# Magicyw/Quadruped-PyMPC-TAMOLS

Hardware: AMD Instinct MI355X
Metric: SRBD rollouts/sec + p50 MPC-step ms at N=10k H=12; 1/2/4/8 GPU (higher is better)
Workload: dtype f32; 1 GPU; go2_trot_flat_mppi_n10000_h12_zo; num_samples=10000, rows_per_gpu=10000, horizon=12, method=mppi, parametrization=zero_order, robot=go2, gait=trot, parallelism=single GPU

## Files before the change

### quadruped-pympc-tamols_amd/csrc/srbd_device.h

```cpp
#pragma once

#include <utility>

#include "srbd_jaxrng.h"
#include "srbd_launch.h"

namespace srbd {

#ifdef SRBD_ROLLOUT_STAMPS
constexpr int RSTAMP_N = 6, RSTAMP_BLOCKS = 8192;
__device__ uint64_t g_rstamp[RSTAMP_BLOCKS * RSTAMP_N];
#define SRBD_RSTAMP(i)                                                                  \
    do {                                                                                \
        if (threadIdx.x == 0 && blockIdx.x < RSTAMP_BLOCKS) {                           \
            asm volatile("s_waitcnt vmcnt(0) lgkmcnt(0)" ::: "memory");                 \
            g_rstamp[blockIdx.x * RSTAMP_N + (i)] = __builtin_amdgcn_s_memrealtime(); \
        }                                                                               \
    } while (0)
__device__ uint64_t g_lstamp[RSTAMP_BLOCKS * 8];
__device__ uint64_t g_fstamp[64];
#define SRBD_LSTAMP(i)                                                                            \
    do {                                                                                          \
        if (threadIdx.x == 0 && blockIdx.x < RSTAMP_BLOCKS)                                       \
            g_lstamp[blockIdx.x * 8 + (i)] = __builtin_amdgcn_s_memrealtime();                    \
// ... 219 lines not shown
    int q = first / n, k = first - q * n;
    const int sq = stride / n, sk = stride - sq * n;
    while (q < nq) {
        rng_item(mc, in->sigma, (uint32_t)seed, (uint32_t)(seed >> 32), (uint32_t)ctr, (uint32_t)(ctr >> 32), k, q,
                 job.noise);
        k += sk;
        q += sq;
        if (k >= n) {
            k -= n;
            ++q;
        }
    }
}

__host__ __device__ constexpr int chunk_index(int n, int H, int S) { return (n * S) / H; }

template <int N>
struct IntC {
    static constexpr int value = N;
};
template <class F, int... Ns>
__device__ __forceinline__ void unroll_seq(F&& f, std::integer_sequence<int, Ns...>) {
    (f(IntC<Ns>{}), ...);
}

__device__ __forceinline__ void st_rec(float* p, float v) {
    __hip_atomic_store(reinterpret_cast<uint32_t*>(p), __float_as_uint(v), __ATOMIC_RELAXED, __HIP_MEMORY_SCOPE_AGENT);
}
__device__ __forceinline__ float ld_rec(const float* p) {
    return __uint_as_float(
        __hip_atomic_load(reinterpret_cast<const uint32_t*>(p), __ATOMIC_RELAXED, __HIP_MEMORY_SCOPE_AGENT));
}
template <int U>
__device__ __forceinline__ void stage_recs16(const float* __restrict__ src, float* dst, int n) {
    const int tid = threadIdx.x, T = blockDim.x, n4 = n >> 2;
    const auto rs = __builtin_amdgcn_make_buffer_rsrc((void*)src, (short)0, n * 4, 0x00020000);
    float4* d4 = reinterpret_cast<float4*>(dst);
    for (int i0 = 0; i0 < n4; i0 += U * T) {
        float4 v[U];
#pragma unroll
        for (int u = 0; u < U; ++u) {
            const auto x = __builtin_amdgcn_raw_buffer_load_b128(rs, 16 * (i0 + u * T + tid), 0, 16);
            v[u] = make_float4(__uint_as_float(x[0]), __uint_as_float(x[1]), __uint_as_float(x[2]),
                               __uint_as_float(x[3]));
        }
#pragma unroll
        for (int u = 0; u < U; ++u) {
            const int i = i0 + u * T + tid;
            if (i < n4) d4[i] = v[u];
        }
    }
}
template <int U>
__device__ __forceinline__ void stage_recs(const float* __restrict__ src, float* dst, int n) {
    const int tid = threadIdx.x, T = blockDim.x, n2 = n >> 1;
    const uint64_t* s2 = reinterpret_cast<const uint64_t*>(src);
    uint64_t* d2 = reinterpret_cast<uint64_t*>(dst);
    for (int i0 = 0; i0 < n2; i0 += U * T) {
        uint64_t v[U];
#pragma unroll
        for (int u = 0; u < U; ++u) {
            const int i = i0 + u * T + tid;
            v[u] = i < n2 ? __hip_atomic_load(s2 + i, __ATOMIC_RELAXED, __HIP_MEMORY_SCOPE_AGENT) : 0ull;
        }
#pragma unroll
        for (int u = 0; u < U; ++u) {
            const int i = i0 + u * T + tid;
            if (i < n2) d2[i] = v[u];
        }
    }
}


__device__ __forceinline__ void fold_node_lds(const ModelConst& mc, const float* st, int rec_stride, int nb, float* G) {
    __shared__ float sc_sh[TREE_FAN];
    __shared__ float gh_sh[2];
    __shared__ uint64_t gk_sh[MAXK + 1];
    const int tid = threadIdx.x, T = blockDim.x;
    const int P = mc.P, K = mc.K;
    const bool rs = mc.method == SRBD_RANDOM_SAMPLING;
    if (tid < 64) {
        const float* R = st + (size_t)tid * rec_stride;
        const bool have = tid < nb;
        const float m = have ? R[0] : 0.0f;
        const uint32_t row = have ? __float_as_uint(R[2]) : 0u;
        const uint64_t key = have ? ((uint64_t)__float_as_uint(m) << 32) | row : KEY_NONE;
        const uint64_t gk = wave_min_u64(key);
        const float beta = __uint_as_float((uint32_t)(gk >> 32));
        if (key == gk) gh_sh[1] = R[3];
        if (tid == 0) {
            gh_sh[0] = beta;
            gk_sh[MAXK] = gk;
        }
        if (have) sc_sh[tid] = rs ? 1.0f : expf(-1.0f * (m - beta));
        if (tid == 0) gk_sh[0] = gk;
    }
    __syncthreads();
    SRBD_LSTAMP(4);
    if (!rs) {
        for (int j = tid; j <= P; j += T) {
            const int off = j < P ? REC_HDR + j : 1;
            float a = 0.0f;
            int cb = 0;
            for (; cb + 8 <= nb; cb += 8) {
                float x[8];
#pragma unroll
                for (int u = 0; u < 8; ++u) x[u] = st[(size_t)(cb + u) * rec_stride + off];
#pragma unroll
                for (int u = 0; u < 8; ++u) a = a + sc_sh[cb + u] * x[u];
            }
            for (; cb < nb; ++cb) a = a + sc_sh[cb] * st[(size_t)cb * rec_stride + off];
            st_rec(&G[off], a);
        }
    }
    SRBD_LSTAMP(5);
    if (tid == 0) {
        st_rec(&G[0], gh_sh[0]);
        if (rs) st_rec(&G[1], 1.0f);
        st_rec(&G[2], __uint_as_float((uint32_t)gk_sh[MAXK]));
        st_rec(&G[3], gh_sh[1]);
    }
    if (tid < K) {
        const uint64_t kk = gk_sh[tid];
        st_rec(&G[REC_HDR + P + 2 * tid], __uint_as_float((uint32_t)kk));
        st_rec(&G[REC_HDR + P + 2 * tid + 1], __uint_as_float((uint32_t)(kk >> 32)));
    }
}

__device__ __forceinline__ bool level1_fold(const ModelConst& mc, const float* __restrict__ recs, int rec_stride,
                                            const GroupArgs& grp, int nroll, int lpb, float* st) {
    __shared__ int last_sh;
    const int tid = threadIdx.x;
    const int bpg = TREE_FAN / lpb;
    const int g = (int)blockIdx.x / bpg;
    const int nblk = min(bpg, nroll - g * bpg);
    const int nb = min(TREE_FAN, mc.nleaf - g * TREE_FAN);
    SRBD_LSTAMP(0);
    asm volatile("s_waitcnt vmcnt(0)" ::: "memory");
    __syncthreads();
    SRBD_LSTAMP(1);
    if (tid == 0) {
        const uint32_t old = __hip_atomic_fetch_add(grp.cnt + g, 1u, __ATOMIC_RELAXED, __HIP_MEMORY_SCOPE_AGENT);
        last_sh = old == (uint32_t)(nblk - 1);
    }
    __syncthreads();
    if (!last_sh) return false;
    SRBD_LSTAMP(2);
    if (tid == 0) __hip_atomic_store(grp.cnt + g, 0u, __ATOMIC_RELAXED, __HIP_MEMORY_SCOPE_AGENT);
    stage_recs16<5>(recs + (size_t)g * TREE_FAN * rec_stride, st, nb * rec_stride);
    __syncthreads();
    SRBD_LSTAMP(3);
    fold_node_lds(mc, st, rec_stride, nb, grp.grecs + (size_t)g * rec_stride);
    return true;
}

template <int CTRL, int ROWMASK>
__device__ __forceinline__ float dpp_f32(float v) {
    return __int_as_float(__builtin_amdgcn_update_dpp(0, __float_as_int(v), CTRL, ROWMASK, 0xF, false));
}
template <int LEVELS>
__device__ __forceinline__ float lane_tree_f32(float v) {
    v = v + dpp_f32<0x111, 0xF>(v);
    v = v + dpp_f32<0x112, 0xF>(v);
    v = v + dpp_f32<0x114, 0xF>(v);
    v = v + dpp_f32<0x118, 0xF>(v);
    if constexpr (LEVELS >= 5) v = v + dpp_f32<0x142, 0xA>(v);
    if constexpr (LEVELS >= 6) v = v + dpp_f32<0x143, 0xC>(v);
    return v;
}
__device__ __forceinline__ float wave_sum_f32(float v) { return lane_tree_f32<6>(v); }

constexpr int REGEN_QUADS = 16;
template <int SPL, int RG>
__device__ __forceinline__ void leaf_wsum_lanes(const ModelConst& mc, const StepInput* __restrict__ in,
                                                const float* __restrict__ base, bool zs, const float* e_sh,
                                                float* rbuf, int rec_stride, int k0, int gen = 0) {
    constexpr int CB = SPL == 4 ? 8 : 12;
    constexpr int LPL = 64 / SPL;
    const int lane = threadIdx.x & 63, w = threadIdx.x >> 6, NW = blockDim.x >> 6;
    const int P = mc.P;
    const size_t ldn = (size_t)mc.ldn;
    float e[SPL];
#pragma unroll
    for (int u = 0; u < SPL; ++u) e[u] = e_sh[SPL * lane + u];
    float* rec = rbuf + (lane / LPL) * rec_stride;
    const bool writer = (lane % LPL) == LPL - 1;
    int jreg = 0;
    if constexpr (RG && SPL == 4) {
        if (RG == 2 || (mc.method == SRBD_MPPI && mc.rng == RNG_PHILOX && in->noise_scaled == 0 && 4 * REGEN_QUADS <= P)) {
            const uint32_t key0 = in->seed_lo, key1 = in->seed_hi, c2 = in->ctr_lo, c3 = in->ctr_hi;
            const int nq = RG == 2 ? gen - 1 : REGEN_QUADS;
            for (int q = w; q < nq; q += NW) {
                float zq[4][SPL];
#pragma unroll
                for (int u = 0; u < SPL; ++u) {
                    const int k = k0 + SPL * lane + u, r = mc.row0 + k;
                    uint32_t c[4] = {(uint32_t)(r - 1), (uint32_t)q, c2, c3};
                    philox4x32_10(c, key0, key1);
                    float v[4];
                    box_muller(c[0], c[1], v[0], v[1]);
                    box_muller(c[2], c[3], v[2], v[3]);
                    const bool live = r > 0 && k < mc.n_local;
#pragma unroll
                    for (int i = 0; i < 4; ++i) zq[i][u] = live ? mc.sigma_mppi * v[i] : 0.0f;
                }
#pragma unroll
                for (int i = 0; i < 4; ++i) {
                    float p[SPL];
#pragma unroll
                    for (int u = 0; u < SPL; ++u) p[u] = e[u] * (zq[i][u] * 1.0f);
                    float a = (p[0] + p[1]) + (p[2] + p[3]);
                    a = lane_tree_f32<4>(a);
                    if (writer) rec[REC_HDR + 4 * q + i] = a;
                }
            }
            jreg = 4 * nq;
        }
    }
    for (int j0 = jreg + w; j0 <= P; j0 += CB * NW) {
        float z[CB][SPL];
#pragma unroll
        for (int b = 0; b < CB; ++b) {
            const int j = j0 + b * NW;
            const float* col = base + (size_t)(j < P ? j : 0) * ldn + SPL * lane;
            if constexpr (SPL == 4) {
                const float4 v = *reinterpret_cast<const float4*>(col);
                z[b][0] = v.x, z[b][1] = v.y, z[b][2] = v.z, z[b][3] = v.w;
            } else {
                const float2 v = *reinterpret_cast<const float2*>(col);
                z[b][0] = v.x, z[b][1] = v.y;
            }
        }
#pragma unroll
        for (int b = 0; b < CB; ++b) {
            const int j = j0 + b * NW;
            if (j > P) break;
            float p[SPL];
            if (j < P) {
                const float sj = zs ? in->sigma[j] : 1.0f;
#pragma unroll
                for (int u = 0; u < SPL; ++u) p[u] = e[u] * (z[b][u] * sj);
            } else {
#pragma unroll
                for (int u = 0; u < SPL; ++u) p[u] = e[u];
            }
            float a;
            if constexpr (SPL == 4)
                a = (p[0] + p[1]) + (p[2] + p[3]);
            else
                a = p[0] + p[1];
            a = lane_tree_f32<SPL == 4 ? 4 : 5>(a);
            if (writer) rec[j < P ? REC_HDR + j : 1] = a;
        }
    }
}

template <bool ZS>
__device__ __forceinline__ void leaf_wsum_cols(const ModelConst& mc, const StepInput* __restrict__ in,
                                               const float* __restrict__ base, const float* zst, int zstride, bool zs,
                                               const float* e_sh, float* __restrict__ rec) {
    const int tid = threadIdx.x, T = blockDim.x, P = mc.P;
    const size_t ldn = (size_t)mc.ldn;
    if ((tid >> 6) == (T >> 6) - 1) {
        const float t = wave_sum_f32(e_sh[tid & 63]);
        if ((tid & 63) == 63) st_rec(&rec[1], t);
    }
    for (int j = tid; j < P; j += T) {
        const float sj = zs ? in->sigma[j] : 1.0f;
        float first = 0.0f, tot = 0.0f;
#pragma nounroll
        for (int h = 0; h < 2; ++h) {
            float lv[16];
            if constexpr (ZS) {
#pragma unroll
                for (int i = 0; i < 16; ++i) {
                    const int r = 32 * h + 2 * i;
                    lv[i] = e_sh[r] * (zst[r * zstride + j] * sj) + e_sh[r + 1] * (zst[(r + 1) * zstride + j] * sj);
                }
            } else {
                const float4* row = reinterpret_cast<const float4*>(base + (size_t)j * ldn) + 8 * h;
                float4 v[8];
#pragma unroll
                for (int i = 0; i < 8; ++i) v[i] = row[i];
#pragma unroll
                for (int i = 0; i < 8; ++i) {
                    const int r = 32 * h + 4 * i;
                    lv[2 * i] = e_sh[r] * (v[i].x * sj) + e_sh[r + 1] * (v[i].y * sj);
                    lv[2 * i + 1] = e_sh[r + 2] * (v[i].z * sj) + e_sh[r + 3] * (v[i].w * sj);
                }
            }
#pragma unroll
            for (int n = 8; n >= 1; n >>= 1)
#pragma unroll
                for (int i = 0; i < n; ++i) lv[i] = lv[2 * i] + lv[2 * i + 1];
            if (h == 0)
                first = lv[0];
            else
                tot = first + lv[0];
        }
        st_rec(&rec[REC_HDR + j], tot);
    }
}

template <bool CEMT, bool ZS = false, bool TF = false, int RG = 0>
__device__ __forceinline__ bool block_epilogue(const ModelConst& mc, const StepInput* __restrict__ in, const int SPB,
                                               int sib, bool valid, float cost, const float* __restrict__ noise,
                                               float* __restrict__ recs, int rec_stride, float tag,
                                               const GroupArgs& grp, int nroll, float* zst = nullptr,
                                               int zstride = 0) {
    __shared__ uint64_t ks[ZS ? 64 : 256];
    __shared__ float e_sh[ZS ? 64 : 256];
    __shared__ uint64_t lmin[4];
    __shared__ uint64_t lel[CEMT ? 4 : 1][CEMT ? MAXK : 1];
    __shared__ float rbuf[TF ? 4 * ((REC_HDR + MAXP + 2 * MAXK + 3) & ~3) : 1];
    const int tid = threadIdx.x, lane = tid & 63, w = tid >> 6;
    const int lpb = SPB >> 6;
    const int P = mc.P, K = mc.K;
    const int k0 = blockIdx.x * SPB;
    const bool rs = mc.method == SRBD_RANDOM_SAMPLING;
    const uint64_t key = (sib >= 0 && valid) ? cost_key(cost, (uint32_t)(mc.row0 + k0 + sib)) : KEY_NONE;
    if (sib >= 0) ks[sib] = key;
    __syncthreads();
    constexpr bool ONE = ZS && !CEMT;
    uint64_t m1 = KEY_NONE;
    if constexpr (ONE) {
        m1 = wave_min_u64(ks[lane]);
    } else if (w < lpb) {
        const uint64_t m = wave_min_u64(ks[64 * w + lane]);
        if (lane == 0) lmin[w] = m;
    }
    if constexpr (CEMT) {
        if (K > 1) {
            for (int i = tid; i < lpb * MAXK; i += (int)blockDim.x) lel[i / MAXK][i % MAXK] = KEY_NONE;
            __syncthreads();
            const int lps = (int)blockDim.x / SPB, part = tid & (lps - 1), s = tid / lps, b = s >> 6;
            const uint64_t mine = ks[s];
            const int span = 64 / lps, i0 = 64 * b + part * span;
            int cnt = 0;
            for (int i = 0; i < span; ++i) cnt += ks[i0 + i] < mine ? 1 : 0;
            if (lps >= 2) cnt += __builtin_amdgcn_mov_dpp(cnt, 0xB1, 0xF, 0xF, true);
            if (lps == 4) cnt += __builtin_amdgcn_mov_dpp(cnt, 0x4E, 0xF, 0xF, true);
            if (part == 0 && cnt < K) lel[b][cnt] = mine;
        }
    }
    if constexpr (!ONE) __syncthreads();
    SRBD_RSTAMP(3);
    if (!rs) {
        const uint64_t lm = ONE ? m1 : (sib >= 0 ? lmin[sib >> 6] : KEY_NONE);
        if (sib >= 0) e_sh[sib] = valid ? expf(-1.0f * (cost - u2f((uint32_t)(lm >> 32)))) : 0.0f;
        __syncthreads();
        const bool zs = CEMT && zs_scaled(mc, in);
        if (SPB == 64)
            leaf_wsum_cols<ZS>(mc, in, noise + k0, zst, zstride, zs, e_sh, recs + (size_t)blockIdx.x * rec_stride);
        else if constexpr (TF) {
            if (SPB == 128)
                leaf_wsum_lanes<2, RG>(mc, in, noise + k0, zs, e_sh, rbuf, rec_stride, k0);
            else
                leaf_wsum_lanes<4, RG>(mc, in, noise + k0, zs, e_sh, rbuf, rec_stride, k0, grp.gen);
        }
    }
    SRBD_RSTAMP(4);
    const bool via_lds = TF && SPB > 64;
    float* const grec = recs + (size_t)blockIdx.x * lpb * rec_stride;
    auto put = [&](int b, int off, float v) {
        if (via_lds)
            rbuf[b * rec_stride + off] = v;
        else
            st_rec(&grec[(size_t)b * rec_stride + off], v);
    };
    auto leafmin = [&](int b) { return ONE ? m1 : lmin[b]; };
    if (tid < lpb) {
        const uint64_t m = leafmin(tid);
        put(tid, 0, u2f((uint32_t)(m >> 32)));
        put(tid, 2, u2f((uint32_t)m));
        if (rs) put(tid, 1, 1.0f);
    }
    if (sib >= 0 && key == leafmin(sib >> 6)) put(sib >> 6, 3, tag);
    for (int i = tid; i < lpb * K; i += (int)blockDim.x) {
        const int b = i / K, q = i % K;
        uint64_t kk = leafmin(b);
        if constexpr (CEMT) kk = K > 1 ? lel[b][q] : kk;
        put(b, REC_HDR + P + 2 * q, u2f((uint32_t)kk));
        put(b, REC_HDR + P + 2 * q + 1, u2f((uint32_t)(kk >> 32)));
    }
    if (via_lds) {
        __syncthreads();
        for (int i = tid; i < lpb * rec_stride; i += (int)blockDim.x) st_rec(&grec[i], rbuf[i]);
    }
    if constexpr (!CEMT) {
        if (grp.gsize > 1) {
            if (grp.fast) return true;
            if constexpr (ZS) {
                return level1_fold(mc, recs, rec_stride, grp, nroll, lpb, zst);
            } else {
                __shared__ __attribute__((aligned(16))) float st[GROUP_LDS_FLOATS];
                return level1_fold(mc, recs, rec_stride, grp, nroll, lpb, st);
            }
        }
    }
    return false;
}

constexpr uint32_t GA_FREQ_LANE = 0x10000u;

__device__ __forceinline__ float ga_sample_freq(const ModelConst& mc, const StepInput* __restrict__ in, int k) {
    if (in->ga_explicit) return mc.ga_freq[k];
    const uint64_t seed = ((uint64_t)in->seed_hi << 32) | in->seed_lo;
    if (mc.rng != RNG_PHILOX)
        return in->ga_freqs[jax_choice_index((uint32_t)(seed >> 32), (uint32_t)seed, (uint64_t)(mc.row0 + k),
                                             (uint64_t)mc.N, (uint32_t)in->ga_nfreq, mc.rng == RNG_JAX)];
    uint32_t c[4] = {(uint32_t)(mc.row0 + k), GA_FREQ_LANE, in->ctr_lo, in->ctr_hi};
    philox4x32_10(c, (uint32_t)seed, (uint32_t)(seed >> 32));
    const uint32_t i = (uint32_t)(((uint64_t)c[0] * (uint32_t)in->ga_nfreq) >> 32);
    return in->ga_freqs[i];
}

__device__ __forceinline__ void ga_contact_masks(const StepInput* __restrict__ in, int H, float f, uint32_t mask[4]) {
    const float inc = in->ga_dt * f;
    float t[4];
#pragma unroll
    for (int l = 0; l < 4; ++l) {
        t[l] = in->ga_timing[l];
        mask[l] = 0u;
    }
    for (int n = 0; n < H; ++n)
#pragma unroll
        for (int l = 0; l < 4; ++l) {
            t[l] = t[l] >= 1.0f ? 0.0f : t[l];
            t[l] = t[l] + inc;
            mask[l] |= (t[l] < in->ga_duty ? 1u : 0u) << n;
        }
}

}
```

### quadruped-pympc-tamols_amd/csrc/srbd_kernels.hip

```cpp
#include "srbd_device.h"
#include "srbd_merge.h"
#include "srbd_quad.h"

#include <cstdlib>

namespace srbd {

__global__ void __launch_bounds__(256) rng_kernel(const ModelConst mc, const StepInput* __restrict__ in,
                                                  const RngJob job) {
    if (job.gate && (*job.gate & ARM_CANCEL)) return;
    rng_items(mc, in, job, blockIdx.x * 256 + threadIdx.x, gridDim.x * 256);
}

__global__ void __launch_bounds__(256) transpose_kernel(const float* __restrict__ src, int n, int P, int ldn,
                                                        float* __restrict__ dst) {
    __shared__ float tile[32][33];
    const int bx = blockIdx.x * 32, by = blockIdx.y * 32;
    const int tx = threadIdx.x & 31, ty = threadIdx.x >> 5;
    for (int i = ty; i < 32; i += 8) {
        const int row = bx + i, col = by + tx;
        tile[i][tx] = (row < n && col < P) ? src[(size_t)row * P + col] : 0.0f;
    }
    __syncthreads();
    for (int i = ty; i < 32; i += 8) {
// ... 18 lines not shown
                                                           const ModelConst mc, const StepInput* __restrict__ in_dev,
                                                           const float* __restrict__ noise, float* __restrict__ costs,
                                                           float* __restrict__ recs, int rec_stride,
    const RngJob next_rng, int nroll, const GroupArgs grp) {
    const StepInput* __restrict__ in;
    if constexpr (KS) {
        (void)ksi;
        const auto ka = (const __attribute__((address_space(4))) StepInput*)__builtin_amdgcn_kernarg_segment_ptr();
        in = (const StepInput*)ka;
        if (blockIdx.x == 0) {
            const auto src = (const __attribute__((address_space(4))) uint32_t*)ka;
            uint32_t* dst = reinterpret_cast<uint32_t*>(const_cast<StepInput*>(in_dev));
            for (int i = threadIdx.x; i < (int)(sizeof(StepInputK) / 4); i += blockDim.x) dst[i] = src[i];
        }
    } else {
        in = in_dev;
    }
    if (grp.gate && (*grp.gate & ARM_CANCEL)) {
        if (FM && blockIdx.x == 0 && threadIdx.x == 0)
            __hip_atomic_store(grp.flag, grp.seq | ARM_CANCEL, __ATOMIC_RELAXED, __HIP_MEMORY_SCOPE_SYSTEM);
        return;
    }
    SRBD_RSTAMP(0);
#if SRBD_PRIO
    if ((int)blockIdx.x < nroll && nroll >= SRBD_PRIO_MIN) __builtin_amdgcn_s_setprio(SRBD_PRIO);
#endif
    if ((int)blockIdx.x >= nroll) {
        rng_items(mc, in, next_rng, ((int)blockIdx.x - nroll) * (int)blockDim.x + (int)threadIdx.x,
                  ((int)gridDim.x - nroll) * (int)blockDim.x);
        SRBD_RSTAMP(5);
        return;
    }

    constexpr bool CT = HT > 0 && (KIND == SRBD_ZERO_ORDER || ST > 0);
    const int SPB = (int)blockDim.x >> 2;
    const int H = CT ? HT : mc.H;
    const int S = CT ? ST : mc.S;
    const int PL = CT ? (KIND == SRBD_ZERO_ORDER ? 3 * HT : (KIND == SRBD_LINEAR_SPLINE ? 3 * (ST + 1) : 12 * ST))
                      : mc.PL;
    constexpr bool ZST = CT && KIND == SRBD_ZERO_ORDER && !EXT && HT <= 12;
    static_assert(!GEN || (ZST && HT % 4 == 0 && !CEMT), "GEN: the zero-order LDS-staged form, H % 4 == 0");
    constexpr int PCT = ZST ? 12 * HT : 1;
    constexpr int ZSTR = PCT + 1;
    __shared__ __attribute__((aligned(16))) float zst[ZST ? (64 * ZSTR > GROUP_LDS_FLOATS ? 64 * ZSTR : GROUP_LDS_FLOATS) : 1];
    __shared__ float bls[ZST ? PCT : 1];
    __shared__ float sls[ZST && CEMT ? PCT : 1];
    const int tid = threadIdx.x;
    const int q4 = tid & 3;
    const int c = q4 < 3 ? q4 : 2;
    const int sib = tid >> 2;
    const int k = blockIdx.x * SPB + sib;
    const bool valid = k < mc.n_local;
    const size_t ldn = (size_t)mc.ldn;
    const float* __restrict__ nz = noise + k;
    const float* __restrict__ best = in->best;
    const bool zs = CEMT && zs_scaled(mc, in);

    const QuadLane L = quad_lane(mc, c);
    const float Qp = sel3(c, mc.Q[0], mc.Q[1], mc.Q[2]), Qv = sel3(c, mc.Q[3], mc.Q[4], mc.Q[5]);
    const float Qr = sel3(c, mc.Q[6], mc.Q[7], mc.Q[8]), Qw = sel3(c, mc.Q[9], mc.Q[10], mc.Q[11]);
    const float* st = in->state;
    const float* rf = in->ref;
    const float rp = sel3(c, rf[0], rf[1], rf[2]), rv = sel3(c, rf[3], rf[4], rf[5]);
    const float rr = sel3(c, rf[6], rf[7], rf[8]), rw = sel3(c, rf[9], rf[10], rf[11]);
    float feet[4];
#pragma unroll
    for (int l = 0; l < 4; ++l) feet[l] = sel3(c, st[12 + 3 * l], st[13 + 3 * l], st[14 + 3 * l]);
    float p = sel3(c, st[0], st[1], st[2]), v = sel3(c, st[3], st[4], st[5]);
    float r = sel3(c, st[6], st[7], st[8]), w = sel3(c, st[9], st[10], st[11]);
    float cost = 0.0f;
    const float rwc = sel3(c, mc.cost_r[0], mc.cost_r[1], mc.cost_r[2]);
    float fprev[4];
    constexpr bool LEGP = !EXT;
    const int lq = q4;
    uint32_t lmask[4];
#pragma unroll
    for (int l = 0; l < 4; ++l) lmask[l] = lq == l ? ~0u : 0u;
    float footL[3];
#pragma unroll
    for (int q = 0; q < 3; ++q) footL[q] = st[12 + 3 * lq + q];
    constexpr int NCL = ZST ? HT : 1;
    float clreg[NCL];
    if constexpr (ZST) {
#pragma unroll
        for (int n = 0; n < HT; ++n) clreg[n] = in->contact[lq][n];
    }

    constexpr int NPRE = !CT ? 1 : (KIND == SRBD_ZERO_ORDER ? HT : (KIND == SRBD_LINEAR_SPLINE ? ST + 1 : 4 * ST));
    float pre[LEGP ? 3 : 4][NPRE];
    const int cblk = LEGP ? lq * PL
                          : (KIND == SRBD_ZERO_ORDER ? c * HT : (KIND == SRBD_LINEAR_SPLINE ? c * (ST + 1) : 4 * c));
    const auto nrs = __builtin_amdgcn_make_buffer_rsrc((void*)noise, (short)0, mc.P * mc.ldn * 4, 0x00020000);
    const int voff = (cblk * mc.ldn + k) * 4;
    const float* __restrict__ bl = best + cblk;
    const float* __restrict__ sl = in->sigma + cblk;
    if constexpr (ZST) {
        for (int j = tid; j < PCT; j += 256) {
            bls[j] = best[j];
            if constexpr (CEMT) sls[j] = in->sigma[j];
        }
    }
    auto load_slot = [&](const int i) __attribute__((always_inline)) {
#pragma unroll
        for (int l = 0; l < (LEGP ? 3 : 4); ++l) {
            const int jr = LEGP ? (KIND == SRBD_ZERO_ORDER ? l * HT + i
                                   : (KIND == SRBD_LINEAR_SPLINE ? l * (ST + 1) + i : 10 * (i >> 2) + 4 * l + (i & 3)))
                                : l * PL + (KIND == SRBD_CUBIC_SPLINE ? 10 * (i >> 2) + (i & 3) : i);
#ifdef SRBD_DIAG_NOLOAD
            const float nzv = (float)(voff + jr * mc.ldn) * 1e-9f;
#else
            const float nzv = __uint_as_float(__builtin_amdgcn_raw_buffer_load_b32(nrs, voff, jr * mc.ldn * 4, 0));
#endif
            if constexpr (ZST) {
                pre[l][i] = nzv;
            } else if constexpr (CEMT) {
                const float sj = sl[jr];
                pre[l][i] = bl[jr] + nzv * (zs ? sj : 1.0f);
            } else {
                pre[l][i] = bl[jr] + nzv;
            }
        }
    };
    constexpr int PW = (EXT && KIND == SRBD_ZERO_ORDER) ? (NPRE < 4 ? NPRE : 4) : NPRE;
    constexpr int CLEAD = 2;
    constexpr bool CWIN = CT && CEMT && KIND == SRBD_CUBIC_SPLINE && ST > 1;
    if constexpr (GEN) {
    } else if constexpr (CWIN) {
#pragma unroll
        for (int i = 0; i < 4; ++i) load_slot(i);
    } else if constexpr (CT) {
#pragma unroll
        for (int i = 0; i < PW; ++i) load_slot(i);
    }
    if constexpr (ZST) {
        asm volatile("s_waitcnt lgkmcnt(0)" ::: "memory");
        __builtin_amdgcn_s_barrier();
    }

    float dep = p;
    auto gen4 = [&](const int s, auto is) __attribute__((always_inline)) {
        const int r = mc.row0 + k;
        const bool live = r > 0 && valid;
        const uint32_t d = (uint32_t)(r - 1);
#pragma unroll
        for (int q = 0; q < 3; ++q) {
            uint32_t cc[4] = {d, (uint32_t)(lq * (PL / 4) + q * (HT / 4) + s), is->ctr_lo, is->ctr_hi};
            philox4x32_10(cc, is->seed_lo, is->seed_hi);
            float v[4];
            box_muller(cc[0], cc[1], v[0], v[1]);
            box_muller(cc[2], cc[3], v[2], v[3]);
#pragma unroll
            for (int i = 0; i < 4; ++i) pre[q][(4 * s + i) % NPRE] = live ? mc.sigma_mppi * v[i] : 0.0f;
        }
    };
    auto step = [&](const int n, auto EX) __attribute__((always_inline)) {
        if constexpr (GEN)
            if (n % 4 == 0) gen4(n / 4, step_ptr(in, cost));
        if constexpr (CT && PW < NPRE)
            if (n + PW < NPRE) load_slot(n + PW);
        if constexpr (CWIN) {
#pragma unroll
            for (int q = 1; q < (CWIN ? ST : 1); ++q) {
                const int at = q * HT / ST - CLEAD;
                if (n == (at > 0 ? at : 0))
#pragma unroll
                    for (int i = 4 * q; i < 4 * q + 4; ++i) load_slot(i);
            }
        }
        const auto is = step_ptr(in, dep);
        float cl[4] = {0.0f, 0.0f, 0.0f, 0.0f};
        if constexpr (!ZST)
#pragma unroll
            for (int l = 0; l < 4; ++l) cl[l] = is->contact[l][n];
        const float fref = is->fzref[n];
        const float dt = mc.dts[n];
        const float sq = mc.sq[n], somq = mc.somq[n], sa = mc.sa[n], sb = mc.sb[n], scc = mc.sc[n], sd = mc.sd[n];
        const int idx = CT && KIND != SRBD_ZERO_ORDER ? chunk_index(n, HT, ST) : mc.sidx[n];
        float temp, temp2, ex = 0.0f;
        if constexpr (LEGP) {
            const float clq = ZST ? clreg[ZST ? n : 0]
                                  : __uint_as_float((__float_as_uint(cl[0]) & lmask[0]) | (__float_as_uint(cl[1]) & lmask[1]) |
                                                    (__float_as_uint(cl[2]) & lmask[2]) | (__float_as_uint(cl[3]) & lmask[3]));
            const int lbase = lq * PL;
            auto PQ = [&](int q, int i, int j) {
                if constexpr (ZST) {
                    if constexpr (CEMT) return bls[lbase + j] + pre[q][i] * (zs ? sls[lbase + j] : 1.0f);
                    return bls[lbase + j] + pre[q][i];
                } else if constexpr (CT) {
                    return pre[q][i];
                } else {
                    const float z = nz[(size_t)(lbase + j) * ldn];
                    return best[lbase + j] + (zs ? z * in->sigma[lbase + j] : z);
                }
            };
            float rq[3];
#pragma unroll
            for (int q = 0; q < 3; ++q) {
                if (KIND == SRBD_ZERO_ORDER) {
                    rq[q] = PQ(q, n, n + q * H);
                } else if (KIND == SRBD_LINEAR_SPLINE) {
                    const int o = idx + q * (S + 1);
                    rq[q] = somq * PQ(q, idx, o) + sq * PQ(q, idx + 1, o + 1);
                } else {
                    const int o = 10 * idx + 4 * q;
                    const float p0 = PQ(q, 4 * idx, o), p1 = PQ(q, 4 * idx + 1, o + 1), p2 = PQ(q, 4 * idx + 2, o + 2),
                                p3 = PQ(q, 4 * idx + 3, o + 3);
                    const float phi = 0.5f * ((p2 - p1) + (p1 - p0));
                    const float phin = 0.5f * ((p3 - p2) + (p2 - p1));
                    rq[q] = sa * p1 + sb * phi + scc * p2 + sd * phin;
                }
            }
            const float fz = clamp_cs((fref + rq[2]) * clq, mc.grf_min, mc.grf_max);
            const float lo = mc.neg_mu * fz, hi = mc.mu * fz;
            const float fx = clamp_cs(third(rq[0] * clq), lo, hi), fy = clamp_cs(third(rq[1] * clq), lo, hi);
            const float vx = footL[0] - qp<QP_B0>(p), vy = footL[1] - qp<QP_B1>(p), vz = footL[2] - qp<QP_B2>(p);
            float sm[6] = {fx * clq, fy * clq, fz * clq, ((-vz) * fy + vy * fz) * clq, (vz * fx + (-vx) * fz) * clq,
                           ((-vy) * fx + vx * fy) * clq};
#pragma unroll
            for (int i = 0; i < 6; ++i) {
                sm[i] = sm[i] + qp<QP_XOR1>(sm[i]);
                sm[i] = sm[i] + qp<QP_XOR2>(sm[i]);
            }
            temp = sel3(c, sm[0], sm[1], sm[2]);
            temp2 = sel3(c, sm[3], sm[4], sm[5]);
            dep = sm[5];
            quad_rb_apply3(mc, L, quad_rb_prep(L, r, w), temp, sm[3], sm[4], sm[5], dt, p, v, r, w);
        } else {
        float tf[4], tt[4];
#pragma unroll
        for (int l = 0; l < 4; ++l) {
            const int base = l * PL;
            auto P = [&](int i, int j) {
                if constexpr (CT) {
                    return pre[l][i];
                } else {
                    const float z = nz[(size_t)(base + j) * ldn];
                    return best[base + j] + (zs ? z * in->sigma[base + j] : z);
                }
            };
            float raw;
            if (KIND == SRBD_ZERO_ORDER) {
                raw = P(n, n + c * H);
            } else if (KIND == SRBD_LINEAR_SPLINE) {
                const int o = idx + c * (S + 1);
                raw = somq * P(idx, o) + sq * P(idx + 1, o + 1);
            } else {
                const int o = 10 * idx + 4 * c;
                const float p0 = P(4 * idx, o), p1 = P(4 * idx + 1, o + 1), p2 = P(4 * idx + 2, o + 2),
                            p3 = P(4 * idx + 3, o + 3);
                const float phi = 0.5f * ((p2 - p1) + (p1 - p0));
                const float phin = 0.5f * ((p3 - p2) + (p2 - p1));
                raw = sa * p1 + sb * phi + scc * p2 + sd * phin;
            }
            float zp = clamp_cs((fref + raw) * cl[l], mc.grf_min, mc.grf_max);
            const float xy = third(raw * cl[l]);
            const float fz = qp<QP_B2>(c == 2 ? zp : xy);
            const float f = c == 2 ? fz : clamp_cs(xy, mc.neg_mu * fz, mc.mu * fz);
            tf[l] = f * cl[l];
            tt[l] = quad_cross(feet[l] - p, f) * cl[l];
            if constexpr (decltype(EX)::value) {
                const float u = c == 2 ? f - (cl[l] != 0.0f ? fref : 0.0f) : f;
                float term = (u * rwc) * u;
                if (n > 0) {
                    const float d = f - fprev[l];
                    term = term + (d * mc.cost_smooth) * d;
                }
                {
                    float vv = fabsf(xy) - mc.mu * fz;
                    vv = vv > 0.0f ? vv : 0.0f;
                    const float cone = (vv * mc.cost_cone) * vv;
                    term = c < 2 ? term + cone : term;
                }
                ex = ex + term;
                fprev[l] = f;
            }
        }
        temp = (tf[0] + tf[1]) + (tf[2] + tf[3]);
        temp2 = (tt[0] + tt[1]) + (tt[2] + tt[3]);
        dep = temp2;
        quad_rigid_body(mc, L, temp, temp2, dt, p, v, r, w);
        }
        const float ep = p - rp, ev = v - rv, er_ = r - rr, ew = w - rw;
        const float tp = (ep * Qp) * ep, tv = (ev * Qv) * ev, tr = (er_ * Qr) * er_, tw = (ew * Qw) * ew;
        cost = cost + (((tp + tv) + tr) + tw);
        if constexpr (decltype(EX)::value) {
            cost = cost + ex;
            asm volatile("" : "+v"(cost));
        }
    };
    auto horizon = [&](auto EX) __attribute__((always_inline)) {
        if constexpr (CT) {
            unroll_seq([&](auto nc) { step(decltype(nc)::value, EX); },
                       std::make_integer_sequence<int, (CT ? HT : 1)>{});
        } else {
            for (int n = 0; n < H; ++n) step(n, EX);
        }
    };
    horizon(std::bool_constant<EXT>{});
    SRBD_RSTAMP(2);
    cost = (qp<QP_B0>(cost) + qp<QP_B1>(cost)) + qp<QP_B2>(cost);
    cost = cost + in->cost_feet;
    if (isnan(cost) || isinf(cost)) cost = 1000000.0f;
    if (valid && q4 == 0 && costs) costs[k] = cost;
    if constexpr (ZST) {
#pragma unroll
        for (int q = 0; q < 3; ++q)
#pragma unroll
            for (int i = 0; i < NPRE; ++i) zst[sib * ZSTR + lq * PL + q * HT + i] = pre[q][i];
    }
#ifdef SRBD_DIAG_NOEPI
    if (tid == 0) recs[blockIdx.x] = cost;
    return;
#endif
    const bool glast = block_epilogue<CEMT, ZST>(mc, in, SPB, q4 == 0 ? sib : -1, valid, cost, noise, recs, rec_stride,
                                                 0.0f, grp, nroll, ZST ? zst : nullptr, ZSTR);
    if constexpr (FM && ZST && !CEMT) {
        if (FM == 1 && grp.fast) {
            if (glast) fast_tail(mc, in, noise, recs, rec_stride, grp, nroll, zst);
        } else if (glast) {
            final_merge<256, FM == 2>(mc, in, noise, rec_stride, grp, zst);
        }
    }
    SRBD_RSTAMP(5);
}

template <int KIND, int HT>
__global__ void __launch_bounds__(512) rollout_ga_quad_kernel(const ModelConst mc, const StepInput* __restrict__ in,
                                                              const float* __restrict__ noise,
                                                              float* __restrict__ costs, float* __restrict__ recs,
                                                              int rec_stride, const RngJob next_rng, int nroll, const GroupArgs grp) {
    if (grp.gate && (*grp.gate & ARM_CANCEL)) return;
    if ((int)blockIdx.x >= nroll) {
        rng_items(mc, in, next_rng, ((int)blockIdx.x - nroll) * (int)blockDim.x + (int)threadIdx.x,
                  ((int)gridDim.x - nroll) * (int)blockDim.x);
        return;
    }
    const int H = HT > 0 ? HT : mc.H, S = mc.S, PL = mc.PL;
    const int tid = threadIdx.x;
    const int q4 = tid & 3;
    const int c = q4 < 3 ? q4 : 2;
    const int sib = tid >> 2;
    const int SPB = (int)blockDim.x >> 2;
    const int k = blockIdx.x * SPB + sib;
    const bool valid = k < mc.n_local;
    const size_t ldn = (size_t)mc.ldn;
    const float* __restrict__ nz = noise + k;
    const float* __restrict__ best = in->best;

    const float f = ga_sample_freq(mc, in, k);
    uint32_t mask[4];
    ga_contact_masks(in, H, f, mask);
    float seg[4];
#pragma unroll
    for (int l = 0; l < 4; ++l) seg[l] = ((float)__popc(mask[l]) + 1.0f) / (float)S;
    int cnt[4] = {-1, -1, -1, -1};

    const QuadLane L = quad_lane(mc, c);
    const float Qp = sel3(c, mc.Q[0], mc.Q[1], mc.Q[2]), Qv = sel3(c, mc.Q[3], mc.Q[4], mc.Q[5]);
    const float Qr = sel3(c, mc.Q[6], mc.Q[7], mc.Q[8]), Qw = sel3(c, mc.Q[9], mc.Q[10], mc.Q[11]);
    const float* st_ = in->state;
    const float* rf = in->ref;
    const float rp = sel3(c, rf[0], rf[1], rf[2]), rv = sel3(c, rf[3], rf[4], rf[5]);
    const float rr = sel3(c, rf[6], rf[7], rf[8]), rw = sel3(c, rf[9], rf[10], rf[11]);
    float feet[4];
#pragma unroll
    for (int l = 0; l < 4; ++l) feet[l] = sel3(c, st_[12 + 3 * l], st_[13 + 3 * l], st_[14 + 3 * l]);
    float p = sel3(c, st_[0], st_[1], st_[2]), v = sel3(c, st_[3], st_[4], st_[5]);
    float r = sel3(c, st_[6], st_[7], st_[8]), w = sel3(c, st_[9], st_[10], st_[11]);
    float cost = 0.0f;
    constexpr int UNR = HT > 0 ? HT : 1;
#pragma unroll UNR
    for (int n = 0; n < H; ++n) {
        float cl[4];
#pragma unroll
        for (int l = 0; l < 4; ++l) {
            const uint32_t b = (mask[l] >> n) & 1u;
            cl[l] = b ? 1.0f : 0.0f;
            cnt[l] += (int)b;
        }
        const float ns = ((cl[0] + cl[1]) + cl[2]) + cl[3];
        const float fref = mc.fz_ns[(int)ns];
        float tf[4], tt[4];
#pragma unroll
        for (int l = 0; l < 4; ++l) {
            const int base = l * PL;
            auto acc = [&](int j) {
                j = j < 0 ? j + PL : j;
                return best[base + j] + nz[(size_t)(base + j) * ldn];
            };
            const int stc = cnt[l];
            float raw;
            if (KIND == SRBD_ZERO_ORDER) {
                raw = acc(stc + c * H);
            } else {
                int idx = 0;
                for (int i = 0; i <= S; ++i)
                    if (stc >= in->ga_cb[i]) idx = i;
                float tau = (float)stc / seg[l];
                tau = tau - (float)idx;
                const float q = tau / 1.0f;
                if (KIND == SRBD_LINEAR_SPLINE) {
                    const float omq = 1.0f - q;
                    const int o = idx + c * (S + 1);
                    raw = omq * acc(o) + q * acc(o + 1);
                } else {
                    const float a = 2.0f * q * q * q - 3.0f * q * q + 1.0f;
                    const float bb = (q * q * q - 2.0f * q * q + q) * 1.0f;
                    const float cc = -2.0f * q * q * q + 3.0f * q * q;
                    const float d = (q * q * q - q * q) * 1.0f;
                    const int o = 10 * idx + 4 * c;
                    const float p0 = acc(o), p1 = acc(o + 1), p2 = acc(o + 2), p3 = acc(o + 3);
                    const float phi = 0.5f * ((p2 - p1) + (p1 - p0));
                    const float phin = 0.5f * ((p3 - p2) + (p2 - p1));
                    raw = a * p1 + bb * phi + cc * p2 + d * phin;
                }
            }
            const float zp = clamp_cs((fref + raw) * cl[l], mc.grf_min, mc.grf_max);
            const float xy = third(raw * cl[l]);
            const float fz = qp<QP_B2>(c == 2 ? zp : xy);
            const float fo = c == 2 ? fz : clamp_cs(xy, mc.neg_mu * fz, mc.mu * fz);
            tf[l] = fo * cl[l];
            tt[l] = quad_cross(feet[l] - p, fo) * cl[l];
        }
        const float temp = (tf[0] + tf[1]) + (tf[2] + tf[3]), temp2 = (tt[0] + tt[1]) + (tt[2] + tt[3]);
        quad_rigid_body(mc, L, temp, temp2, mc.dts[n], p, v, r, w);
        const float ep = p - rp, ev = v - rv, er_ = r - rr, ew = w - rw;
        const float tp = (ep * Qp) * ep, tv = (ev * Qv) * ev, tr = (er_ * Qr) * er_, tw = (ew * Qw) * ew;
        cost = cost + (((tp + tv) + tr) + tw);
    }
    cost = (qp<QP_B0>(cost) + qp<QP_B1>(cost)) + qp<QP_B2>(cost);
    cost = cost + in->cost_feet;
    const float df = f - 1.3f;
    cost = cost + (df * 100.0f) * df;
    if (isnan(cost) || isinf(cost)) cost = 1000000.0f;
    if (valid && q4 == 0 && costs) costs[k] = cost;
    block_epilogue<false>(mc, in, SPB, q4 == 0 ? sib : -1, valid, cost, noise, recs, rec_stride, f, grp, nroll);
}


template <int NT, bool STAGE>
__global__ void __launch_bounds__(NT) merge_kernel(const ModelConst mc, StepInput* __restrict__ in,
                                                              const float* __restrict__ recs, int nrec,
                                                              int rec_stride, int rows_in_rec,
                                                              const float* __restrict__ noise,
                                                              float* __restrict__ rank_out,
                                                              StepOutput* __restrict__ out, int chain,
                                                              int ctr_inc, uint64_t* __restrict__ dbg,
                                                              uint32_t* __restrict__ flag, uint32_t seq,
                                                              int split_cs, int fence_sys,
                                                              const uint32_t* __restrict__ gate, int levels_up) {
    if (gate && (*gate & ARM_CANCEL)) {
        if (threadIdx.x == 0 && flag)
            __hip_atomic_store(flag + (split_cs > 0 ? blockIdx.x : 0), seq | ARM_CANCEL, __ATOMIC_RELAXED,
                               __HIP_MEMORY_SCOPE_SYSTEM);
        return;
    }
    __shared__ MergeShared<NT> sh;
    extern __shared__ __attribute__((aligned(16))) float dsm[];
    merge_body<NT, STAGE, true>(mc, in, recs, nrec, rec_stride, rows_in_rec, noise, rank_out, out, chain, ctr_inc, dbg, flag,
                          seq, split_cs, fence_sys, sh, dsm, false, levels_up, reinterpret_cast<SplitXchg*>(in + 1));
}

template <int NT>
__device__ __forceinline__ bool xchg_exchange(const XchgArgs& x, const float* mine, StepOutput* out, uint32_t* flag,
                                              uint32_t seq) {
    const int tid = threadIdx.x, T = NT;
    const int stride = x.stride;
    const uint32_t epoch = *x.epoch + 1;
    const size_t half = (size_t)(epoch & 1u) * x.world * stride;
    for (int i = tid; i < (x.world - 1) * stride; i += T) {
        const int q = i / stride, k = i - q * stride;
        const int p = q < x.rank ? q : q + 1;
        __hip_atomic_store(reinterpret_cast<uint32_t*>(x.peer_mailbox[p]) + half + (size_t)x.rank * stride + k,
                           __float_as_uint(mine[k]), __ATOMIC_RELAXED, __HIP_MEMORY_SCOPE_SYSTEM);
    }
    asm volatile("s_waitcnt vmcnt(0)" ::: "memory");
    __syncthreads();
    if (tid < x.world && tid != x.rank) {
        __threadfence_system();
        asm volatile("s_waitcnt vmcnt(0)" ::: "memory");
        __hip_atomic_store(x.peer_flags[tid] + x.rank, epoch, __ATOMIC_RELAXED, __HIP_MEMORY_SCOPE_SYSTEM);
    }
    __shared__ int timed_out;
    if (tid == 0) timed_out = 0;
    __syncthreads();
    if (tid < x.world && tid != x.rank) {
        const uint64_t t0 = __builtin_amdgcn_s_memrealtime();
        while ((int32_t)(__hip_atomic_load(x.flags + tid, __ATOMIC_RELAXED, __HIP_MEMORY_SCOPE_SYSTEM) - epoch) < 0) {
            __builtin_amdgcn_s_sleep(2);
            if (__builtin_amdgcn_s_memrealtime() - t0 > XCHG_TIMEOUT_TICKS) {
                timed_out = 1;
                break;
            }
        }
    }
    __syncthreads();
    if (tid == 0) *x.epoch = epoch;
    if (timed_out) {
        if (tid == 0) {
            *x.err = 1;
            if (out) out->status = -1;
            __threadfence_system();
            if (flag) __hip_atomic_store(flag, seq, __ATOMIC_RELAXED, __HIP_MEMORY_SCOPE_SYSTEM);
        }
        return false;
    }
    for (int i = tid; i < (x.world - 1) * stride; i += T) {
        const int q = i / stride, k = i - q * stride;
        const size_t o = (size_t)(q < x.rank ? q : q + 1) * stride + k;
        x.stage[o] = __uint_as_float(__hip_atomic_load(reinterpret_cast<const uint32_t*>(x.mailbox) + half + o,
                                                       __ATOMIC_RELAXED, __HIP_MEMORY_SCOPE_SYSTEM));
    }
    __syncthreads();
    return true;
}
template <int NT, bool STAGE1>
__global__ void __launch_bounds__(NT) merge_xchg_kernel(const ModelConst mc, StepInput* __restrict__ in,
                                                        const float* __restrict__ recs, int nrec, int rec_stride,
                                                        const float* __restrict__ noise, XchgArgs x,
                                                        StepOutput* __restrict__ out, int chain, int ctr_inc,
                                                        uint32_t* __restrict__ flag, uint32_t seq, int levels_up) {
    __shared__ MergeShared<NT> sh;
    extern __shared__ __attribute__((aligned(16))) float dsm[];
    float* mine = x.stage + (size_t)x.rank * x.stride;
    merge_body<NT, STAGE1>(mc, in, recs, nrec, rec_stride, 0, noise, mine, nullptr, 0, 0, nullptr, nullptr, 0, 0, 1, sh,
                           dsm, false, levels_up);
    __syncthreads();
    if (!xchg_exchange<NT>(x, mine, out, flag, seq)) return;
    merge_body<NT, false>(mc, in, x.stage, mc.t_xnodes, rec_floats_rank(mc.P, mc.K), 1, noise, nullptr, out, chain,
                          ctr_inc, nullptr, flag, seq, 0, 1, sh, dsm);
}



template <int NT, bool XG>
__device__ void final_merge(const ModelConst& mc, const StepInput* in, const float* noise, int rec_stride,
                            const GroupArgs& grp, float* lds) {
    __shared__ int fin;
#ifdef SRBD_ROLLOUT_STAMPS
    const uint64_t f1 = __builtin_amdgcn_s_memrealtime();
#endif
    asm volatile("s_waitcnt vmcnt(0)" ::: "memory");
    __syncthreads();
#ifdef SRBD_ROLLOUT_STAMPS
    const uint64_t f2 = __builtin_amdgcn_s_memrealtime();
#endif
    if (threadIdx.x == 0) {
        const uint32_t old = __hip_atomic_fetch_add(grp.gdone, 1u, __ATOMIC_RELAXED, __HIP_MEMORY_SCOPE_AGENT);
        fin = old == (uint32_t)(grp.ngroups - 1);
    }
    __syncthreads();
    if (!fin) return;
    uint64_t* dbg = nullptr;
#ifdef SRBD_ROLLOUT_STAMPS
    if (threadIdx.x == 0) {
        g_fstamp[0] = blockIdx.x + 1;
        g_fstamp[1] = f1;
        g_fstamp[2] = f2;
        g_fstamp[3] = __builtin_amdgcn_s_memrealtime();
    }
    dbg = g_fstamp + 32;
#endif
    if (threadIdx.x == 0) __hip_atomic_store(grp.gdone, 0u, __ATOMIC_RELAXED, __HIP_MEMORY_SCOPE_AGENT);
    MergeShared<NT>& sh = *reinterpret_cast<MergeShared<NT>*>(lds);
    float* smem = lds + (sizeof(MergeShared<NT>) + 15) / 16 * 4;
    stage_recs16<5>(grp.grecs, smem, grp.ngroups * rec_stride);
    __syncthreads();
#ifdef SRBD_ROLLOUT_STAMPS
    if (threadIdx.x == 0) g_fstamp[4] = __builtin_amdgcn_s_memrealtime();
#endif
    int nrec = grp.ngroups, stride = rec_stride;
    for (int pass = 0;; ++pass) {
        const bool rank_pass = XG && pass == 0;
        float* mine = rank_pass ? grp.xa->stage + (size_t)grp.xa->rank * grp.xa->stride : nullptr;
        merge_body<NT, true>(mc, const_cast<StepInput*>(in), smem, nrec, stride, 0, noise, mine,
                             rank_pass ? nullptr : grp.out, 0, 0, rank_pass ? nullptr : dbg,
                             rank_pass ? nullptr : grp.flag, grp.seq, 0,
                             grp.fence_sys, sh, smem, true, rank_pass ? grp.levels_up : 0);
        if (!rank_pass) return;
        __syncthreads();
        if (!xchg_exchange<NT>(*grp.xa, mine, grp.out, grp.flag, grp.seq)) return;
        nrec = mc.t_xnodes;
        stride = rec_floats_rank(mc.P, mc.K);
        for (int i = threadIdx.x; i < nrec * stride; i += NT) smem[i] = grp.xa->stage[i];
        __syncthreads();
    }
}

size_t final_merge_lds(const ModelConst& mc, int ngroups, int rec_stride) {
    const size_t a = sizeof(float) * (size_t)ngroups * rec_stride + merge_smem_bytes(ngroups, mc.P, mc.K);
    const size_t b =
        sizeof(float) * (size_t)mc.t_xnodes * rec_floats_rank(mc.P, mc.K) + merge_smem_bytes(mc.t_xnodes, mc.P, mc.K);
    return (sizeof(MergeShared<256>) + 15) / 16 * 16 + (a > b ? a : b);
}

__device__ __forceinline__ uint64_t tag_word(uint32_t seq, float v) { return ((uint64_t)seq << 32) | f2u(v); }
__device__ __forceinline__ void st_tag(uint64_t* p, uint64_t w) {
    __hip_atomic_store(p, w, __ATOMIC_RELAXED, __HIP_MEMORY_SCOPE_AGENT);
}
__device__ __forceinline__ void st_sys(void* p, float v) {
    __hip_atomic_store(reinterpret_cast<uint32_t*>(p), __float_as_uint(v), __ATOMIC_RELAXED, __HIP_MEMORY_SCOPE_SYSTEM);
}
constexpr int FT_TAIL0 = 192;
__host__ __device__ constexpr int ft_lds_floats(int P, int rec_stride) {
    return TREE_FAN * rec_stride + ((P + 3) & ~3) + ((P + 4) & ~3) + 4 * 40 + 2 * 4 * 64;
}
__device__ __forceinline__ void ft_prep(const ModelConst& mc, const StepInput* in, float* tsh, float& b0,
                                        float& state_hi) {
    const int tid = threadIdx.x, P = mc.P;
    const auto gin = (const __attribute__((address_space(1))) StepInput*)in;
    if (tid >= FT_TAIL0 && tid < FT_TAIL0 + 4) {
        const int qc = tid - FT_TAIL0 < 3 ? tid - FT_TAIL0 : 2;
        float tail_pre[13];
        merge_tail_load(gin, qc, tail_pre);
        merge_tail_lane(mc, qc, tail_pre, tsh + 40 * (tid - FT_TAIL0));
    }
    if (tid < P) b0 = gin->best[tid];
    if (tid >= 12 && tid < 24) state_hi = gin->state[tid];
// ... 621 lines not shown
```

Measured before the change: 448.8 million rollouts/s.

## Compute MPPI leaf weighted sums from registers via DPP reductions

For the MPPI zero-order path, the per-sample weighted control sums are now computed directly from register-held parameters. Each value is multiplied by its exp weight and reduced across lanes with DPP row shifts. Per-group partials go to LDS, and a 16-way tree sum writes them to the record. This replaces writing every sample's parameters to the zst scratch and re-reading them column-wise, cutting shared-memory traffic and a pass in the epilogue. The cost is more register pressure and the assumption of a fixed 16-group lane layout.

```diff
diff --git a/quadruped-pympc-tamols_amd/csrc/srbd_device.h b/quadruped-pympc-tamols_amd/csrc/srbd_device.h
--- a/quadruped-pympc-tamols_amd/csrc/srbd_device.h
+++ b/quadruped-pympc-tamols_amd/csrc/srbd_device.h
@@ -545,12 +545,52 @@
     }
 }
 
-template <bool CEMT, bool ZS = false, bool TF = false, int RG = 0>
+template <int HT>
+__device__ __forceinline__ void leaf_wsum_regs(const float* pre, float e, float* xch, float* __restrict__ rec) {
+    constexpr int P = 12 * HT, XS = P + 1;
+    const int tid = threadIdx.x, lq = tid & 3;
+    const bool writer = (tid & 12) == 12;
+    float* xr = xch + (tid >> 4) * XS + lq * 3 * HT;
+#pragma unroll
+    for (int q = 0; q < 3; ++q) {
+        float t[HT];
+#pragma unroll
+        for (int i = 0; i < HT; ++i) {
+            t[i] = e * pre[q * HT + i];
+            t[i] = t[i] + dpp_f32<0x114, 0xF>(t[i]);
+            t[i] = t[i] + dpp_f32<0x118, 0xF>(t[i]);
+        }
+        if (writer) {
+#pragma unroll
+            for (int i = 0; i < HT; ++i) {
+                asm volatile("" : "+v"(t[i]));
+                xr[q * HT + i] = t[i];
+            }
+        }
+    }
+    float es = e + dpp_f32<0x114, 0xF>(e);
+    es = es + dpp_f32<0x118, 0xF>(es);
+    if (writer && lq == 0) xch[(tid >> 4) * XS + P] = es;
+    __syncthreads();
+    if (tid <= P) {
+        float lv[16];
+#pragma unroll
+        for (int i = 0; i < 16; ++i) lv[i] = xch[i * XS + tid];
+#pragma unroll
+        for (int n = 8; n >= 1; n >>= 1)
+#pragma unroll
+            for (int i = 0; i < n; ++i) lv[i] = lv[2 * i] + lv[2 * i + 1];
+        st_rec(&rec[tid < P ? REC_HDR + tid : 1], lv[0]);
+    }
+}
+
+template <bool CEMT, bool ZS = false, bool TF = false, int RG = 0, int NR = 0>
 __device__ __forceinline__ bool block_epilogue(const ModelConst& mc, const StepInput* __restrict__ in, const int SPB,
                                                int sib, bool valid, float cost, const float* __restrict__ noise,
                                                float* __restrict__ recs, int rec_stride, float tag,
                                                const GroupArgs& grp, int nroll, float* zst = nullptr,
-                                               int zstride = 0) {
+                                               int zstride = 0, const float* pre = nullptr) {
+    static_assert(NR == 0 || (ZS && !CEMT), "register leaf sums: one leaf per block, MPPI / random sampling");
     __shared__ uint64_t ks[ZS ? 64 : 256];
     __shared__ float e_sh[ZS ? 64 : 256];
     __shared__ uint64_t lmin[4];
@@ -588,7 +628,12 @@
     }
     if constexpr (!ONE) __syncthreads();
     SRBD_RSTAMP(3);
-    if (!rs) {
+    if constexpr (NR > 0) {
+        if (!rs) {
+            const float e = valid ? expf(-1.0f * (cost - u2f((uint32_t)(m1 >> 32)))) : 0.0f;
+            leaf_wsum_regs<NR>(pre, e, zst, recs + (size_t)blockIdx.x * rec_stride);
+        }
+    } else if (!rs) {
         const uint64_t lm = ONE ? m1 : (sib >= 0 ? lmin[sib >> 6] : KEY_NONE);
         if (sib >= 0) e_sh[sib] = valid ? expf(-1.0f * (cost - u2f((uint32_t)(lm >> 32)))) : 0.0f;
         __syncthreads();
diff --git a/quadruped-pympc-tamols_amd/csrc/srbd_kernels.hip b/quadruped-pympc-tamols_amd/csrc/srbd_kernels.hip
--- a/quadruped-pympc-tamols_amd/csrc/srbd_kernels.hip
+++ b/quadruped-pympc-tamols_amd/csrc/srbd_kernels.hip
@@ -344,7 +344,8 @@
     cost = cost + in->cost_feet;
     if (isnan(cost) || isinf(cost)) cost = 1000000.0f;
     if (valid && q4 == 0 && costs) costs[k] = cost;
-    if constexpr (ZST) {
+    constexpr int NR = ZST && !CEMT ? NPRE : 0;
+    if constexpr (ZST && CEMT) {
 #pragma unroll
         for (int q = 0; q < 3; ++q)
 #pragma unroll
@@ -354,8 +355,9 @@
     if (tid == 0) recs[blockIdx.x] = cost;
     return;
 #endif
-    const bool glast = block_epilogue<CEMT, ZST>(mc, in, SPB, q4 == 0 ? sib : -1, valid, cost, noise, recs, rec_stride,
-                                                 0.0f, grp, nroll, ZST ? zst : nullptr, ZSTR);
+    const bool glast = block_epilogue<CEMT, ZST, false, 0, NR>(mc, in, SPB, q4 == 0 ? sib : -1, valid, cost, noise, recs,
+                                                               rec_stride, 0.0f, grp, nroll, ZST ? zst : nullptr, ZSTR,
+                                                               &pre[0][0]);
     if constexpr (FM && ZST && !CEMT) {
         if (FM == 1 && grp.fast) {
             if (glast) fast_tail(mc, in, noise, recs, rec_stride, grp, nroll, zst);
```

New measurement: 443.0 million rollouts/s. 1.3% lower.
